# osmocom/osmo-trx

Hardware: AMD Instinct MI355X
Metric: Mbursts/s detect+demod (156.25 sym, 4 SPS) (higher is better)
Workload: dtype f32

## Files before the change

osmo_trx_amd/csrc/trx_capi.cpp:

```cpp
#include <hip/hip_runtime.h>

#include <cmath>
#include <cstdio>
#include <cstdlib>
#include <cstring>
#include <new>
#include <vector>

#include "../../include/trxhip.h"
#include "trx_tables.h"
#include "trx_ctx.h"
#include "trx_launch.h"

extern "C" {

int trxhip_abi_version(void) { return TRXHIP_ABI_VERSION; }

int trxhip_device_count(void)
{
	int n = 0;
	if (hipGetDeviceCount(&n) != hipSuccess)
		return 0;
	return n;
}
// ... 51 lines not shown
	hipDeviceProp_t prop;
	if (hipGetDeviceProperties(&prop, device) != hipSuccess)
		return TRXHIP_ENODEV;

	trxhip_ctx *ctx = new (std::nothrow) trxhip_ctx;
	if (!ctx)
		return TRXHIP_ENOMEM;
	ctx->device = device;
	ctx->n_cu = prop.multiProcessorCount > 0 ? prop.multiProcessorCount : 256;
	ctx->no_unit = trx_unit_masks_match(t) ? 0 : 1;
	ctx->sch_unit = trx_unit_mask_sch_match(t) ? 1 : 0;
	ctx->pool_enabled = getenv("TRXHIP_NO_POOL") ? 0 : 1;
	ctx->nb_enabled = getenv("TRXHIP_NO_NB_KERNEL") ? 0 : 1;
	for (int k = 0; k < 8; k++)
		if (memcmp(&t->dec_taps[k], &t->dec_taps[15 - k], sizeof(float)) != 0)
			ctx->no_sym = 1;
	for (int f = 0; f < 512 && !ctx->no_fast; f++) {
		double sum = 0.0;
		for (int k = 0; k < 8; k++) {
			const int qa = 512 * k + f, qb = 512 * k + (512 - f);
			sum += fabs((double)t->sincv[trx_sincv_swz(qa)]);
			if (qb < TRX_SINCV_LEN)
				sum += fabs((double)t->sincv[trx_sincv_swz(qb)]);
		}
		if (!(sum <= 2.6))
			ctx->no_fast = 1;
	}
	int rc = TRXHIP_OK;
	if (hipMalloc(reinterpret_cast<void **>(&ctx->d_tables), sizeof(trx_tables)) != hipSuccess) {
		ctx->d_tables = nullptr;
		rc = TRXHIP_ENOMEM;
	} else if (hipMemcpy(ctx->d_tables, h_blob, sizeof(trx_tables), hipMemcpyHostToDevice) != hipSuccess) {
		rc = TRXHIP_EIO;
	} else if (!ctx->redo.create()) {
		rc = TRXHIP_ENOMEM;
	} else {
		trx_tx_tables *tx = static_cast<trx_tx_tables *>(malloc(sizeof(trx_tx_tables)));
		if (!tx || trx_tx_tables_generate(tx) != 0)
			rc = TRXHIP_ENOMEM;
		else if (hipMalloc(reinterpret_cast<void **>(&ctx->d_tx_tables), sizeof(trx_tx_tables)) != hipSuccess) {
			ctx->d_tx_tables = nullptr;
			rc = TRXHIP_ENOMEM;
		} else if (hipMemcpy(ctx->d_tx_tables, tx, sizeof(trx_tx_tables), hipMemcpyHostToDevice) != hipSuccess) {
			rc = TRXHIP_EIO;
		}
		free(tx);
	}
	if (rc != TRXHIP_OK) {
		trxhip_destroy(ctx);
		return rc;
	}
	if (hipMalloc(reinterpret_cast<void **>(&ctx->d_pool), TRX_POOL_SLOTS * 64) != hipSuccess ||
	    hipMemset(ctx->d_pool, 0, TRX_POOL_SLOTS * 64) != hipSuccess) {
		if (ctx->d_pool) (void)hipFree(ctx->d_pool);
		ctx->d_pool = nullptr;
	}
	*out = ctx;
	return TRXHIP_OK;
}

int trxhip_create(trxhip_ctx **out, int device)
{
	if (!out)
		return TRXHIP_EINVAL;
	trx_tables *t = static_cast<trx_tables *>(malloc(sizeof(trx_tables)));
	if (!t)
		return TRXHIP_ENOMEM;
	int rc = trx_tables_generate(t) == 0 ? TRXHIP_OK : TRXHIP_EINVAL;
	if (rc == TRXHIP_OK)
		rc = trxhip_create_from_tables(out, device, t, sizeof(trx_tables));
	free(t);
	return rc;
}

void trxhip_destroy(trxhip_ctx *ctx)
{
	if (!ctx)
		return;
	if (hipSetDevice(ctx->device) == hipSuccess) {
		if (ctx->d_tables) (void)hipFree(ctx->d_tables);
		if (ctx->d_pool) (void)hipFree(ctx->d_pool);
		if (ctx->d_tx_tables) (void)hipFree(ctx->d_tx_tables);
		for (float *t : ctx->d_rs_resamp)
			if (t) (void)hipFree(t);
		ctx->redo.destroy();
	}
	delete ctx;
}

int trxhip_set_nb_kernel(trxhip_ctx *ctx, int enabled)
{
	if (!ctx)
		return TRXHIP_EINVAL;
	ctx->nb_enabled = enabled ? 1 : 0;
	return TRXHIP_OK;
}

int trxhip_set_work_pool(trxhip_ctx *ctx, int enabled)
{
	if (!ctx)
		return TRXHIP_EINVAL;
	ctx->pool_enabled = enabled ? 1 : 0;
	return TRXHIP_OK;
}

int trxhip_fast_stats(trxhip_ctx *ctx, uint64_t *out4, int reset)
{
	if (!ctx || !out4)
		return TRXHIP_EINVAL;
	if (with_device(ctx))
		return TRXHIP_EIO;
	unsigned long long v[4] = { 0, 0, 0, 0 };
	if (trx_fast_stats_read(v, reset) != 0)
// ... 89 lines not shown
		return TRXHIP_EIO;
	if (flags & ~(TRXHIP_FLAG_SLICE | TRXHIP_FLAG_EXACT_DEMOD | TRXHIP_FLAG_IDLE_DUMMY | TRXHIP_FLAG_FEW_NB_SLOTS))
		return TRXHIP_EINVAL;
	const bool few_nb = (flags & TRXHIP_FLAG_FEW_NB_SLOTS) != 0;
	flags &= ~TRXHIP_FLAG_FEW_NB_SLOTS;
	if (ctx->no_unit)
		flags |= TRX_IFLAG_NO_UNIT;
	if (ctx->no_sym)
		flags |= TRX_IFLAG_NO_SYM;
	if (ctx->no_fast)
		flags |= TRX_IFLAG_NO_FAST;
	const hipStream_t st = static_cast<hipStream_t>(stream);

	hipStreamCaptureStatus cap = hipStreamCaptureStatusNone;
	const bool capturing = st && hipStreamIsCapturing(st, &cap) == hipSuccess && cap != hipStreamCaptureStatusNone;
	const bool exact = (flags & TRXHIP_FLAG_EXACT_DEMOD) != 0;
	const bool k4 = sps == 4 && burst_len >= 624 && burst_len <= 628;
	const bool common = k4 && burst_len == 625 && d_soft && !d_ebp_in && soft_stride == 148 &&
			    (flags & ~TRXHIP_FLAG_EXACT_DEMOD) == TRXHIP_FLAG_SLICE && !(cf32 && exact);
	const bool split = common && !cf32 && !exact && ctx->nb_enabled && !few_nb && !capturing;
	unsigned *pool = nullptr;
	if (k4 && ctx->d_pool && ctx->pool_enabled && !capturing && n_bursts >= (size_t)ctx->n_cu * 128)
		pool = ctx->d_pool + (size_t)(ctx->pool_next.fetch_add(1u, std::memory_order_relaxed) % TRX_POOL_SLOTS) * 16;

	if (!k4) {
		const int nld = sps == 1 ? 3 : burst_len <= 640 ? 10 : 0;
		return trx_launch_pull(d_iq, cf32, nld, d_params, d_results, d_soft, ctx->d_tables, d_ebp_in, n_bursts, burst_len, sps,
				       threshold, full_scale, soft_stride, flags, ctx->n_cu, st);
	}
	if (split) {
		std::lock_guard<std::mutex> lk(ctx->redo.mu);
		if (trx_redo_lists::slot *sl = ctx->redo.acquire(n_bursts, st)) {
			const int rc = trx_launch_pull4_nb(pool, d_iq, d_params, d_results, d_soft, ctx->d_tables, n_bursts, threshold,
							   full_scale, ctx->n_cu, sl->d, sl->h_left, st);
			ctx->redo.launched(*sl, rc, st);
			return rc;
		}
	}
	return trx_launch_pull4(pool, d_iq, cf32, exact, common, d_params, d_results, d_soft, ctx->d_tables, d_ebp_in, n_bursts,
				burst_len, threshold, full_scale, soft_stride, flags, ctx->n_cu, st);
}

int trxhip_select_diversity_batch(trxhip_ctx *ctx, const int16_t *d_iq_paths, size_t n_bursts, int n_paths, int burst_len, int sps,
				  int16_t *d_iq_sel, float *d_avg_energy, uint8_t *d_path, void *stream)
{
	if (!ctx || n_paths < 1 || n_paths > 8 || (sps != 1 && sps != 4) || burst_len < 1 || burst_len > TRXHIP_MAX_BURST_LEN)
		return TRXHIP_EINVAL;
	{
		const int window = 20 * sps < burst_len ? 20 * sps : burst_len;
		if (4 * (window - 1) >= burst_len)
			return TRXHIP_EINVAL;
	}
	if (n_bursts == 0)
		return TRXHIP_OK;
	if (!d_iq_paths || !d_iq_sel || !d_avg_energy || (reinterpret_cast<uintptr_t>(d_iq_paths) & 3) ||
	    (reinterpret_cast<uintptr_t>(d_iq_sel) & 3))
		return TRXHIP_EINVAL;
	if (with_device(ctx))
		return TRXHIP_EIO;
	return trx_launch_diversity_select(d_iq_paths, n_bursts, n_paths, burst_len, sps, d_iq_sel, d_avg_energy, d_path,
					   static_cast<hipStream_t>(stream));
}

int trxhip_apply_diversity_power(trxhip_ctx *ctx, trxhip_burst_result *d_results, const trxhip_burst_params *d_params,
				 const float *d_avg_energy, size_t n_bursts, float full_scale, void *stream)
{
	if (!ctx || !(full_scale > 0.0f))
// ... 614 lines not shown
```

osmo_trx_amd/csrc/trx_ctx.h:

```cpp
#ifndef TRX_CTX_H
#define TRX_CTX_H
#include <hip/hip_runtime.h>
#include <atomic>
#include <mutex>
#include "../../include/trxhip.h"
#include "trx_tables.h"
#include "trx_tx_tables.h"

#define TRX_POOL_SLOTS 1024
#define TRX_REDO_SLOTS 4

struct trx_redo_lists {
	struct slot {
		unsigned *d = nullptr;
		size_t cap = 0;
		hipEvent_t ev = nullptr;
		bool busy = false;
		unsigned *h_left = nullptr;
		size_t n_last = 0;
	};
	std::mutex mu;
	slot s[TRX_REDO_SLOTS];
	unsigned next = 0;
	unsigned backoff = 0;
// ... 31 lines not shown
			if (hipMalloc(reinterpret_cast<void **>(&sl.d), bytes) != hipSuccess || hipMemsetAsync(sl.d, 0, bytes, stream) != hipSuccess) {
				if (sl.d) (void)hipFree(sl.d);
				sl.d = nullptr;
				return nullptr;
			}
			sl.cap = cap;
		}
		return &sl;
	}
	void launched(slot &sl, int rc, hipStream_t stream)
	{
		if (rc != 0)
			return;
		if (hipEventRecord(sl.ev, stream) == hipSuccess)
			sl.busy = true;
		else
			(void)hipStreamSynchronize(stream);
	}
	void destroy()
	{
		for (slot &sl : s) {
			if (sl.busy) (void)hipEventSynchronize(sl.ev);
			if (sl.ev) (void)hipEventDestroy(sl.ev);
			if (sl.d) (void)hipFree(sl.d);
			if (sl.h_left) (void)hipHostFree(sl.h_left);
		}
	}
};

struct trxhip_ctx {
	int device = 0;
	int n_cu = 0;
	trx_tables *d_tables = nullptr;
	int no_unit = 0;
	int sch_unit = 0;
	int no_sym = 0;
	int no_fast = 0;
	unsigned *d_pool = nullptr;
	int pool_enabled = 1;
	std::atomic<unsigned> pool_next{0u};
	int nb_enabled = 1;
	trx_redo_lists redo;
	trx_tx_tables *d_tx_tables = nullptr;
	std::mutex tx_mu;
	double tx_full_scale = 0.0;
	bool tx_att_valid = false;
	float tx_att_scale[256];
	std::mutex rs_mu;
	float *d_rs_resamp[2] = { nullptr, nullptr };
};

static inline int with_device(const trxhip_ctx *ctx)
{
	return hipSetDevice(ctx->device) == hipSuccess ? 0 : TRXHIP_EIO;
}
#endif
```

osmo_trx_amd/csrc/trx_kernel4.hip:

```cpp
#include <atomic>
#include "trx_device.h"
#include "trx_launch.h"

#include "trx_k4_common.h"

#define K4_CZ_LEN (TRX_CZ_PAD + TRX_CORR_NARROW + TRX_CZ_PAD)
#define K4_SLICE (K4_XS + TRX_DEC_NARROW + K4_CZ_LEN)
#define K4_DROWS (TRX_DELAY_FILTS + 1)
#define K4_PKC_INTS (5 * WAVE)
#define K4_TABLES_FLOATS (TRX_SINCV_LDS + K4_DROWS * TRX_DELAY_HLEN + 2 * 160 + 16 + 2 * LSEQ_TAPS + 8 * LSEQ_NHDR + K4_DROWS * 36 + K4_PKC_INTS)
#define K4_TABLES_BYTES (K4_TABLES_FLOATS * 4)
#define K4_POOL_RING 64
#define K4_POOL_UNSET (-1)
#define K4_POOL_END (-2)
#define K4_NO_BURST 0xffffffffu
#define K4_LDS_TAIL (16 + 4 * K4_POOL_RING)


#ifdef TRX_DIAG
extern "C" int trxhip_diag_read(unsigned long long *out, int reset)
{
	static unsigned long long h[TRX_DIAG_WAVES * 24];
	if (hipMemcpyFromSymbol(h, HIP_SYMBOL(g_trx_diag), sizeof(h)) != hipSuccess) return -1;
	for (int k = 0; k < 32; k++) out[k] = 0;
// ... 895 lines not shown
	DIAG_FLUSH();
}

extern "C" int trx_fast_stats_read(unsigned long long *out4, int reset)
{
	if (hipMemcpyFromSymbol(out4, HIP_SYMBOL(g_trx_fast_stats), 4 * sizeof(unsigned long long)) != hipSuccess)
		return -1;
	if (reset) {
		const unsigned long long z[4] = { 0, 0, 0, 0 };
		if (hipMemcpyToSymbol(HIP_SYMBOL(g_trx_fast_stats), z, sizeof(z)) != hipSuccess)
			return -1;
	}
	return 0;
}

extern "C" int trx_unit_masks_match(const trx_tables *t)
{
	static const unsigned long long want[12] = { TRX_UNIT_NEG_TSC0, TRX_UNIT_NEG_TSC1, TRX_UNIT_NEG_TSC2, TRX_UNIT_NEG_TSC3,
						     TRX_UNIT_NEG_TSC4, TRX_UNIT_NEG_TSC5, TRX_UNIT_NEG_TSC6, TRX_UNIT_NEG_TSC7,
						     TRX_UNIT_NEG_RACH0, TRX_UNIT_NEG_RACH1, TRX_UNIT_NEG_RACH2, TRX_UNIT_NEG_DUMMY };
	for (int s = 0; s < 12; s++)
		if (!((t->unit_ok >> s) & 1u) || t->unit_neg[s] != want[s])
			return 0;
	return 1;
}

#include "trx_kernel_nb.hip"

static inline size_t k4_lds_bytes(bool cf32, bool exact)
{
	return K4_TABLES_BYTES + (size_t)K4_WPB(cf32, exact) * K4_SLICE * sizeof(c32) + K4_LDS_TAIL;
}

extern "C" int trx_launch_pull4_nb(unsigned *d_pool_ctr, const void *d_iq, const trxhip_burst_params *d_params,
				   trxhip_burst_result *d_results, float *d_soft, const trx_tables *d_tab, size_t n_bursts,
				   float thresh, float full_scale, int n_cu, unsigned *d_redo, unsigned *h_left, hipStream_t stream)
{
	if (n_bursts == 0)
		return 0;
	const size_t grid = trx_burst_grid(n_bursts, (size_t)n_cu);
	{
		constexpr auto k = nb_pull4_kernel;
		if (trx_arm_dynamic_lds<k>())
			return TRXHIP_EIO;
		hipLaunchKernelGGL(k, dim3((unsigned)grid), dim3(NB_WPB * WAVE), NB_LDS_BYTES, stream, reinterpret_cast<const uint32_t *>(d_iq),
				   d_params, d_results, d_soft, d_tab, (unsigned)n_bursts, thresh, full_scale, d_pool_ctr, d_redo,
				   thresh * thresh * 0.2f, thresh * thresh * (1.0f / 6.0f), thresh * thresh * (1.0f / 7.0f), thresh * thresh * 0.125f);
	}
	{
		constexpr auto k = burst_pull4_kernel<false, false, true, true>;
		if (trx_arm_dynamic_lds<k>())
			return TRXHIP_EIO;
		hipLaunchKernelGGL(k, dim3((unsigned)n_cu), dim3(K4_WPB(false, false) * WAVE), k4_lds_bytes(false, false), stream, d_iq, d_params,
				   d_results, d_soft, d_tab, (const float4 *)nullptr, (unsigned)n_bursts, 625, thresh, full_scale, 148,
				   TRXHIP_FLAG_SLICE, h_left, d_redo);
	}
	return hipGetLastError() == hipSuccess ? 0 : TRXHIP_EIO;
}

extern "C" int trx_launch_pull4(unsigned *d_pool_ctr, const void *d_iq, int cf32, int exact, int common, const trxhip_burst_params *d_params,
				trxhip_burst_result *d_results, float *d_soft, const trx_tables *d_tab, const float *d_ebp_in, size_t n_bursts,
				int L, float thresh, float full_scale, int soft_stride, int flags, int n_cu, hipStream_t stream)
{
	if (n_bursts == 0)
		return 0;
	const size_t grid = trx_burst_grid(n_bursts, (size_t)n_cu);
	const size_t lds = k4_lds_bytes(cf32, exact);
#define LAUNCH4(CF_, EX_, CM_)                                                                                  \
	do {                                                                                                    \
		constexpr auto k = burst_pull4_kernel<CF_, EX_, CM_>;                                           \
		if (trx_arm_dynamic_lds<k>((int)lds))                                                           \
			return TRXHIP_EIO;                                                                      \
		hipLaunchKernelGGL(k, dim3((unsigned)grid), dim3(K4_WPB(CF_, EX_) * WAVE), lds, stream,         \
				   d_iq, d_params, d_results, d_soft, d_tab, reinterpret_cast<const float4 *>(d_ebp_in), \
				   (unsigned)n_bursts, L, thresh, full_scale, soft_stride, flags, d_pool_ctr, (unsigned *)nullptr); \
	} while (0)
	if (cf32)        { if (exact) LAUNCH4(true, true, false); else if (common) LAUNCH4(true, false, true); else LAUNCH4(true, false, false); }
	else if (common) { if (exact) LAUNCH4(false, true, true); else LAUNCH4(false, false, true); }
	else             { if (exact) LAUNCH4(false, true, false); else LAUNCH4(false, false, false); }
#undef LAUNCH4
// ... 3 lines not shown
```

osmo_trx_amd/csrc/trx_kernel_nb.hip:

```cpp
#include "trx_k4_common.h"
#include "trx_nb_asm.inc"

#define NB_D_LEN    160
#define NB_CZ_LEN   (TRX_CZ_PAD + TRX_CORR_NARROW + TRX_CZ_PAD)
#define NB_SLICE    (K4_XS + NB_D_LEN + NB_CZ_LEN)
#define NB_COMP_ROWS (TRX_DELAY_FILTS + 1)
#define NB_TABLES_FLOATS (TRX_SINCV_LDS + 16 * WAVE + NB_COMP_ROWS * 36 + 16 + 8 * 8 + 5 * WAVE + 5 * WAVE + 2 * 8 * 16)
#define NB_TABLES_BYTES (NB_TABLES_FLOATS * 4)
#define NB_WPB 16
#define NB_POOL_RING 64
#define NB_POOL_UNSET (-1)
#define NB_POOL_END (-2)
#define NB_NO_BURST 0xffffffffu
#define NB_LDS_TAIL (16 + 4 * NB_POOL_RING)
#define NB_LDS_BYTES (NB_TABLES_BYTES + NB_WPB * NB_SLICE * 8 + NB_LDS_TAIL)
#define NB_MAX_TOA 32



typedef float v3f __attribute__((ext_vector_type(3)));
typedef int v4i __attribute__((ext_vector_type(4)));

template <typename T>
__device__ __forceinline__ unsigned lds_addr(const T *p)
{
	return (unsigned)(uintptr_t)(const __attribute__((address_space(3))) T *)p;
}

__global__ void __launch_bounds__(NB_WPB * WAVE)
nb_pull4_kernel(const uint32_t *__restrict__ iq, const trxhip_burst_params *__restrict__ params,
		trxhip_burst_result *__restrict__ results, float *__restrict__ soft, const trx_tables *__restrict__ tab,
		unsigned n_bursts, float thresh, float full_scale, unsigned *__restrict__ pool_ctr, unsigned *__restrict__ redo,
		float gk5, float gk6, float gk7, float gk8)
{
	static_assert(NB_TABLES_BYTES % 16 == 0 && (NB_SLICE * 8) % 16 == 0 && (K4_XS * 8) % 16 == 0 && (NB_D_LEN * 8) % 16 == 0, "16-byte LDS accesses");
	static_assert(NB_LDS_BYTES <= 160 * 1024, "LDS");
	static_assert(NB_ASM_GDEC_OFF == (TRX_SINCV_LDS + 16 * WAVE + NB_COMP_ROWS * 36) * 4, "tools/gen_nb_asm.py: LDS offset of the decimator taps");
	static_assert(NB_ASM_DEC_MAX_NACT == 15 + NB_ASM_CORR_MAX_LEN, "tools/gen_nb_asm.py: DEC and CORR change form at the same window");
	static_assert(NB_ASM_LSEQ_OFF == (NB_TABLES_FLOATS - 2 * 8 * 16) * 4, "tools/gen_nb_asm.py: LDS offset of the training-sequence taps");
	constexpr int NLD = 10;
	extern __shared__ __attribute__((aligned(16))) char smem[];
	const int lane0 = threadIdx.x & (WAVE - 1);
	const int wave = uni((int)(threadIdx.x >> 6));

	float *const sincv = reinterpret_cast<float *>(smem);
	float *const wa4f = sincv + TRX_SINCV_LDS;
	const float4 *const wa4 = reinterpret_cast<const float4 *>(wa4f);
	float *const comp = wa4f + 16 * WAVE;
	float *const gdec = comp + NB_COMP_ROWS * 36;
	float *const lhdr = gdec + 16;
	int *const pkcl = reinterpret_cast<int *>(lhdr + 8 * 8);
	int *const lcn = pkcl + 5 * WAVE;
	c32 *const lseq = reinterpret_cast<c32 *>(lcn + 5 * WAVE);
	c32 *const wbase = reinterpret_cast<c32 *>(smem + NB_TABLES_BYTES) + (size_t)wave * NB_SLICE;
	int *const wg_next = reinterpret_cast<int *>(reinterpret_cast<c32 *>(smem + NB_TABLES_BYTES) + (size_t)NB_WPB * NB_SLICE);
	int *const pool_g = wg_next + 4;
	c32 *const P = wbase;
	c32 *const D = wbase + K4_XS;
	c32 *const cz = D + NB_D_LEN + TRX_CZ_PAD;

	for (int i = threadIdx.x; i < TRX_SINCV_LDS; i += blockDim.x)
		sincv[i] = (i < TRX_SINCV_LEN) ? tab->sincv[i] : 0.0f;
	for (int i = threadIdx.x; i < 16 * WAVE; i += blockDim.x) {
		const int l = i & (WAVE - 1), u = i >> 6;
		const PeakConst pcl = peak_const(l);
		const int q = (u < 8) ? pcl.loA + 512 * (7 - u) : pcl.hiA + 512 * (u - 8);
		wa4f[((u >> 2) * WAVE + l) * 4 + (u & 3)] = (q < TRX_SINCV_LEN) ? tab->sincv[q] : 0.0f;
	}
	for (int i = threadIdx.x; i < NB_COMP_ROWS * 36; i += blockDim.x) {
		const int f = i / 36, j = i % 36;
		comp[i] = (j >= TRX_FUSED_SH) ? tab->comp_filt[f][j - TRX_FUSED_SH] : 0.0f;
	}
	if (threadIdx.x < 16)
		gdec[threadIdx.x] = tab->dec_taps[threadIdx.x];
	if (threadIdx.x < 128)
		lseq[threadIdx.x] = make_float2(tab->seq[TRX_SEQ_TSC0 + (threadIdx.x >> 4)].taps[threadIdx.x & 15].re,
						tab->seq[TRX_SEQ_TSC0 + (threadIdx.x >> 4)].taps[threadIdx.x & 15].im);
	if (threadIdx.x < 64)
		lhdr[threadIdx.x] = reinterpret_cast<const float *>(&tab->seq[TRX_SEQ_TSC0 + (threadIdx.x >> 3)].gain)[threadIdx.x & 7];
	if (threadIdx.x < WAVE) {
		const PeakConst pc0 = peak_const(threadIdx.x);
		pkcl[0 * WAVE + threadIdx.x] = pc0.flA;
		pkcl[1 * WAVE + threadIdx.x] = pc0.loA;
		pkcl[2 * WAVE + threadIdx.x] = pc0.hiA;
		pkcl[3 * WAVE + threadIdx.x] = pc0.offB;
		pkcl[4 * WAVE + threadIdx.x] = pc0.ratio_off;
		lcn[0 * WAVE + threadIdx.x] = pc0.ratio_off * 8;
		lcn[1 * WAVE + threadIdx.x] = (pc0.flA - 8) * 8;
		lcn[2 * WAVE + threadIdx.x] = pc0.offB;
		const int l = threadIdx.x, e = (l - 52) / 3, t = (l - 52) % 3;
		const bool sp = l >= 52;
		lcn[3 * WAVE + l] = 8 * (sp ? (t == 0 ? e : t == 1 ? e + 3 : e - 3) : 4 + 3 * (l < 49 ? l : 49));
		lcn[4 * WAVE + l] = sp ? (e + (t == 2 ? 4 : 0)) * K4_NTP * 4 : -1;
	}
	for (int i = lane0; i < NB_SLICE; i += WAVE)
		wbase[i] = make_float2(0.0f, 0.0f);
	if (threadIdx.x == 0) {
		wg_next[0] = NB_WPB;
		wg_next[1] = 0;
	}
	if (threadIdx.x < NB_POOL_RING)
		pool_g[threadIdx.x] = NB_POOL_UNSET;
	__syncthreads();

	const float fs_db = 6.02059991f * __log2f(full_scale);
	const float thr2 = thresh * thresh;
	const float gc0 = thr2 * 1.0001e-5f;
	int t5pk = 0;
	bool t5_ok = true;
	for (int t = 0; t < 8; t++) {
		const int v = (int)(lhdr[8 * t + 5] * 512.0f);
		t5_ok = t5_ok && v >= -8 && v <= 7 && (float)v == lhdr[8 * t + 5] * 512.0f;
		t5pk |= (v & 15) << (4 * t);
	}
	t5pk = uni(t5pk);
	const unsigned long long e8_addr = reinterpret_cast<unsigned long long>(&tab->edge8[0][0][0]);
	const unsigned n_wg = gridDim.x;
	const unsigned n_groups = (n_bursts + 15u) >> 4;
	const bool pooled = pool_ctr != nullptr;
	const unsigned n_static_groups = pooled ? ((n_groups - (n_groups >> 3)) / n_wg) * n_wg : n_groups;
	const unsigned n_pool_groups = n_groups - n_static_groups;
	const unsigned gq = n_static_groups / n_wg, gr = n_static_groups % n_wg;
	const unsigned my_groups = gq + (blockIdx.x < gr ? 1u : 0u);
	const unsigned base16 = (blockIdx.x * gq + (blockIdx.x < gr ? blockIdx.x : gr)) << 4;
	unsigned items = my_groups << 4;
	if (base16 + items > n_bursts)
		items = (base16 < n_bursts) ? n_bursts - base16 : 0u;
	auto burst_of = [&](unsigned jj) -> unsigned {
		if (jj < items)
			return base16 + jj;
		if (!pooled)
			return NB_NO_BURST;
		const unsigned k = (jj - items) >> 4;
		volatile int *slot = pool_g + (k & (NB_POOL_RING - 1));
		int g;
		while ((g = *slot) == NB_POOL_UNSET)
			__builtin_amdgcn_s_sleep(2);
		g = uni(g);
		if (g < 0)
			return NB_NO_BURST;
		const unsigned bb = ((n_static_groups + (unsigned)g) << 4) + (jj & 15u);
		return bb < n_bursts ? bb : NB_NO_BURST;
	};
	auto pool_draw = [&](unsigned jj, bool ended, int lane) {
		const unsigned k = (jj + 16u - items) >> 4;
		int g = NB_POOL_END;
		if (!ended) {
			unsigned p = 0;
			if (lane == 0)
				p = __hip_atomic_fetch_add(pool_ctr, 1u, __ATOMIC_RELAXED, __HIP_MEMORY_SCOPE_AGENT);
			p = (unsigned)uni((int)p);
			g = (p < n_pool_groups) ? (int)p : NB_POOL_END;
		}
		if (lane == 0) {
			pool_g[(k + NB_POOL_RING / 2) & (NB_POOL_RING - 1)] = NB_POOL_UNSET;
			pool_g[k & (NB_POOL_RING - 1)] = g;
		}
	};

	uint32_t pre_i[NLD];
	uint32_t pre_prm = 0u;
	auto prefetch = [&](unsigned bb, int lane) {
		pre_prm = reinterpret_cast<const uint32_t *>(params)[2 * (size_t)bb];
		const uint32_t *src = iq + (size_t)bb * 625;
		const unsigned ul = (unsigned)lane & 63u;
#pragma unroll
		for (int r = 0; r < NLD - 1; r++)
			pre_i[r] = __builtin_nontemporal_load(src + (unsigned)(r * WAVE) + ul);
		pre_i[NLD - 1] = __builtin_nontemporal_load(src + (unsigned)((NLD - 1) * WAVE) + min(ul, 48u));
	};
	const unsigned b_first = burst_of((unsigned)wave);
	if (b_first != NB_NO_BURST)
		prefetch(b_first, lane0);

	v3f o = { 0.0f, 0.0f, 0.0f };
	int recw = 0;
	bool pend_any = false;
	bool pend_rec = false;
	unsigned pend_b = 0;
	bool left_any = false;
	int q_xr = 0, q_xi = 0, q_es = 0, q_toa = 0, q_s = 0, q_fl = 0, q_b = 0;
	int q_n = 0;
	auto flush_records = [&](const int lane) {
		if (lane < q_n) {
			const float *const h = lhdr + 8 * (q_fl & 0xff);
			const float xr = __int_as_float(q_xr), xi = __int_as_float(q_xi);
			const float a0 = xr * h[2], a1 = xr * h[3], a2 = xi * h[3], a3 = xi * h[2];
			const float amp_re = a0 - a2, amp_im = a1 + a3;
			const float toa = (float)q_toa * 0.001953125f;
			const float energy = __int_as_float(q_es) * 0.0125f;
			const float rssi = fs_db - 3.01029996f * __log2f(energy);
			const float p2 = xi * xi + xr * xr;
			const float C = p2 * h[7];
			const float S = __int_as_float(q_s);
			const float ci = 3.0103f * __log2f(C * __builtin_amdgcn_rcpf(S - C));
			const v4i r0 = { 1, __float_as_int(toa), __float_as_int(amp_re), __float_as_int(amp_im) };
			const v4i r1 = { __float_as_int(ci), __float_as_int(energy), __float_as_int(rssi), q_fl };
			asm volatile("global_store_dwordx4 %0, %1, off\n\t"
				     "global_store_dwordx4 %0, %2, off offset:16\n\t"
				     "s_nop 1"
				     :: "v"(results + (unsigned)q_b), "v"(r0), "v"(r1) : "memory");
		}
		q_n = 0;
	};

	auto demod_general = [&](const int nk, const c32 ampv, const int lane) -> bool {
// ... 87 lines not shown
				dec[hi_i] = cmul(make_float2(sr, si), scale);
		}
		wave_sync();
		auto pick = [&](int i) {
			const float d = reinterpret_cast<const float *>(dec + i)[i & 1];
			return __builtin_amdgcn_fmed3f(fmaf((i & 2) ? -0.5f : 0.5f, d, 0.5f), 0.0f, 1.0f);
		};
		const bool reg = lane >= 2 && lane < 50;
		const int i0 = reg ? 3 * lane - 2 : ((((lane - 54) * 11) >> 5) & 3);
		o.x = pick(i0);
		o.y = pick(reg ? i0 + 1 : 0);
		o.z = pick(reg ? i0 + 2 : 0);
		wave_sync();
		return true;
	};

	DIAG_DECL;
	unsigned j_next = 0, b_next = NB_NO_BURST;
	for (unsigned b = b_first; b != NB_NO_BURST; b = b_next) {
		int lane;
		asm volatile("v_mbcnt_lo_u32_b32 %0, -1, 0\n\tv_mbcnt_hi_u32_b32 %0, -1, %0" : "=v"(lane));
		const int ticket = claim_issue(wg_next);
		const unsigned prm0 = (unsigned)uni((int)pre_prm);
		const unsigned max_toa = prm0 >> 16;
		const int tsc = (prm0 >> 8) & 0xff;
		bool leave = ((prm0 & 0xf8ffu) != (unsigned)TRXHIP_TSC) || (max_toa > NB_MAX_TOA) || !t5_ok;

		c32 *const pload = P + (lane & 3) * PH_A + PH_M0 + (lane >> 2);
		float amax = 0.0f, epart = 0.0f;
#ifdef TRX_DIAG
		DIAG_MARK(12);
		asm volatile("s_waitcnt vmcnt(0)" ::: "memory");
		DIAG_MARK(13);
#endif
		if (!leave) {
#pragma unroll
			for (int r = 0; r < NLD; r++) {
				const int i = r * WAVE + lane;
				if (r < NLD - 1 || i < 625) {
					const c32 v = make_float2((float)(int16_t)(pre_i[r] & 0xffffu), (float)(int16_t)(pre_i[r] >> 16));
					pload[16 * r] = v;
					asm("v_max3_f32 %0, %0, |%1|, |%2|" : "+v"(amax) : "v"(v.x), "v"(v.y));
					if (r < 5)
						epart = fmaf(v.x, v.x, fmaf(v.y, v.y, epart));
				}
			}
		} else {
#pragma unroll
			for (int r = 0; r < NLD; r++)
				asm volatile("" :: "v"(pre_i[r]));
		}
		DIAG_MARK(14);
		if (pend_any) {
			float *const so = soft + (size_t)pend_b * 148;
			int *const rp = reinterpret_cast<int *>(results + pend_b);
			const float oe = o.x;
			asm volatile("s_bfm_b64 exec, 48, 2\n\t"
				     "global_store_dwordx3 %0, %1, %2 offset:16\n\t"
				     "s_mov_b32 exec_lo, 0\n\t"
			     "s_mov_b32 exec_hi, 0x92400000\n\t"
				     "global_store_dword %3, %4, %2\n\t"
				     "s_mov_b64 exec, %8\n\t"
				     "global_store_dword %5, %6, %7\n\t"
				     "s_mov_b64 exec, -1\n\t"
				     "s_nop 0"
				     :: "v"((lane - 2) * 12), "v"(o), "s"(so), "v"((((lane - 54) * 11) >> 5) * 4), "v"(oe), "v"(lane * 4), "v"(recw), "s"(rp),
// ... 159 lines not shown
			continue;
		}
		pend_b = b;
		pend_any = true;
		if (q_n == WAVE)
			flush_records(lane);
		DIAG_MARK(11);
	}
	if (pend_any) {
		int lane;
		asm volatile("v_mbcnt_lo_u32_b32 %0, -1, 0\n\tv_mbcnt_hi_u32_b32 %0, -1, %0" : "=v"(lane));
		float *const so = soft + (size_t)pend_b * 148;
		int *const rp = reinterpret_cast<int *>(results + pend_b);
		const float oe = o.x;
		asm volatile("s_bfm_b64 exec, 48, 2\n\t"
			     "global_store_dwordx3 %0, %1, %2 offset:16\n\t"
		     "s_mov_b32 exec_lo, 0\n\t"
		     "s_mov_b32 exec_hi, 0x92400000\n\t"
			     "global_store_dword %3, %4, %2\n\t"
			     "s_mov_b64 exec, %8\n\t"
			     "global_store_dword %5, %6, %7\n\t"
			     "s_mov_b64 exec, -1\n\t"
			     "s_nop 0"
			     :: "v"((lane - 2) * 12), "v"(o), "s"(so), "v"((((lane - 54) * 11) >> 5) * 4), "v"(oe), "v"(lane * 4), "v"(recw), "s"(rp),
			        "s"(pend_rec ? 0xffull : 0ull)
			     : "memory");
	}
	{
		int lane;
		asm volatile("v_mbcnt_lo_u32_b32 %0, -1, 0\n\tv_mbcnt_hi_u32_b32 %0, -1, %0" : "=v"(lane));
		flush_records(lane);
	}
	DIAG_FLUSH();
	if (pooled) {
		__syncthreads();
		int tid0;
		asm volatile("v_mbcnt_lo_u32_b32 %0, -1, 0\n\tv_mbcnt_hi_u32_b32 %0, -1, %0" : "=v"(tid0));
		if (tid0 == 0 && atomicAdd(wg_next + 1, 1) == 0) {
			const unsigned d = __hip_atomic_fetch_add(pool_ctr + 1, 1u, __ATOMIC_ACQ_REL, __HIP_MEMORY_SCOPE_AGENT);
			if (d == gridDim.x - 1u) {
				__hip_atomic_store(pool_ctr, 0u, __ATOMIC_RELAXED, __HIP_MEMORY_SCOPE_AGENT);
				__hip_atomic_store(pool_ctr + 1, 0u, __ATOMIC_RELEASE, __HIP_MEMORY_SCOPE_AGENT);
			}
		}
	}
}
```

osmo_trx_amd/csrc/trx_launch.h:

```cpp
#ifndef TRX_LAUNCH_H
#define TRX_LAUNCH_H
#include <hip/hip_runtime.h>
#include <stdint.h>
#include "../../include/trxhip.h"
#include "trx_tables.h"
#include "trx_tx_tables.h"

constexpr int trx_arfcn_pchan(int rows, int l)
{
	return rows == 4 ? l : (rows == 1 ? 0 : (rows == 2 ? (l == 0 ? 0 : 3) : (l == 0 ? 1 : (l == 1 ? 0 : 3))));
}

extern "C" {


int trx_launch_pull4(unsigned *d_pool_ctr, const void *d_iq, int cf32, int exact, int common, const trxhip_burst_params *d_params,
		     trxhip_burst_result *d_results, float *d_soft, const trx_tables *d_tab, const float *d_ebp_in, size_t n_bursts,
		     int L, float thresh, float full_scale, int soft_stride, int flags, int n_cu, hipStream_t stream);
int trx_launch_pull4_nb(unsigned *d_pool_ctr, const void *d_iq, const trxhip_burst_params *d_params, trxhip_burst_result *d_results,
			float *d_soft, const trx_tables *d_tab, size_t n_bursts, float thresh, float full_scale, int n_cu,
			unsigned *d_redo, unsigned *h_left, hipStream_t stream);
int trx_launch_pull(const void *d_iq, int cf32, int nld, const trxhip_burst_params *d_params, trxhip_burst_result *d_results,
		    float *d_soft, const trx_tables *d_tab, const float *d_ebp_in, size_t n_bursts, int L, int sps, float thresh,
		    float full_scale, int soft_stride, int flags, int n_cu, hipStream_t stream);
size_t trx_pull_lds_bytes(int L, int waves_per_block);

int trx_fast_stats_read(unsigned long long *out4, int reset);
int trx_unit_masks_match(const trx_tables *t);
int trx_unit_mask_sch_match(const trx_tables *t);

int trx_launch_sch_detect(const float *d_iq, size_t buf_stride, trxhip_burst_result *d_results, const trx_tables *d_tab,
			  size_t n_bufs, int len, int start, int toa_sub, float thresh, int unit_tables, hipStream_t stream);
size_t trx_va_lds_bytes(int L);
int trx_launch_va_demod(const float *d_iq, const trxhip_burst_params *d_params, const trxhip_burst_result *d_detected, float *d_soft,
			int32_t *d_starts, size_t n_bursts, int L, float scale, int soft_stride, int flags, hipStream_t stream);

int trx_launch_pack_trxd(const trxhip_burst_result *d_results, const float *d_soft, int soft_stride, uint8_t *d_pkt,
			 size_t n_bursts, float rssi_offset, hipStream_t stream);
int trx_launch_pack_trxd_wire(const trxhip_burst_result *d_results, const trxhip_burst_params *d_params, const float *d_soft,
			      int soft_stride, const trxhip_trxd_meta *d_meta, uint8_t *d_pkt, int pkt_stride, uint16_t *d_pkt_len,
			      size_t n_bursts, float rssi_offset, hipStream_t stream, trxhip_burst_result *d_results_copy);
int trx_launch_gather_bursts(const unsigned long long *d_src, void *d_dst, size_t n, unsigned dwords, hipStream_t stream);
int trx_launch_convolve(const float *d_x, int x_len, const float *d_h, int h_len, int h_complex, float *d_y, int y_len, int start,
			int len, size_t n_vec, hipStream_t stream);
int trx_launch_convert_short_float(float *d_out, const int16_t *d_in, size_t len, hipStream_t stream);
int trx_launch_convert_float_short(int16_t *d_out, const float *d_in, float scale, size_t len, hipStream_t stream);
int trx_launch_dft_strided(const float *d_in, float *d_out, int m, size_t howmany, size_t istride, size_t ostride, int reverse,
			   hipStream_t stream);
int trx_launch_energy_detect(const float *d_x, size_t n_bursts, int burst_len, unsigned window, float *d_out, hipStream_t stream);
int trx_launch_diversity_select(const int16_t *d_iq_paths, size_t n_bursts, int n_paths, int burst_len, int sps, int16_t *d_iq_sel,
				float *d_avg_energy, uint8_t *d_path, hipStream_t stream);
int trx_launch_diversity_power(trxhip_burst_result *d_res, const trxhip_burst_params *d_params, const float *d_avg_energy,
			       size_t n_bursts, float full_scale, hipStream_t stream);
int trx_launch_delay_vector(const float *d_in, float *d_out, const float *d_delays, const trx_tables *d_tab, size_t n_vec, int len,
// ... 39 lines not shown
```

Baseline: 1079.

## Precompute NB kernel LDS table image once and bulk-copy it per workgroup

Builds the narrowband kernel's LDS table block once at context creation by running a one-off staging kernel and saving the result to a device buffer. Each workgroup of the NB kernel then loads that image with three 16-byte loads per thread and stores it to LDS while the first burst's prefetch is in flight, so the per-element table construction and the t5 packing loop no longer run in every block. This costs an extra device buffer and changes the launch signature. The NB path now fails with EINVAL if the image is missing.

```diff
diff --git a/osmo_trx_amd/csrc/trx_capi.cpp b/osmo_trx_amd/csrc/trx_capi.cpp
--- a/osmo_trx_amd/csrc/trx_capi.cpp
+++ b/osmo_trx_amd/csrc/trx_capi.cpp
@@ -107,6 +107,7 @@
 		rc = TRXHIP_ENOMEM;
 	} else if (hipMemcpy(ctx->d_tables, h_blob, sizeof(trx_tables), hipMemcpyHostToDevice) != hipSuccess) {
 		rc = TRXHIP_EIO;
+	} else if ((rc = trx_nb_lds_image_create(ctx->d_tables, &ctx->d_nb_lds)) != TRXHIP_OK) {
 	} else if (!ctx->redo.create()) {
 		rc = TRXHIP_ENOMEM;
 	} else {
@@ -154,6 +155,7 @@
 		return;
 	if (hipSetDevice(ctx->device) == hipSuccess) {
 		if (ctx->d_tables) (void)hipFree(ctx->d_tables);
+		if (ctx->d_nb_lds) (void)hipFree(ctx->d_nb_lds);
 		if (ctx->d_pool) (void)hipFree(ctx->d_pool);
 		if (ctx->d_tx_tables) (void)hipFree(ctx->d_tx_tables);
 		for (float *t : ctx->d_rs_resamp)
@@ -309,7 +311,7 @@
 		std::lock_guard<std::mutex> lk(ctx->redo.mu);
 		if (trx_redo_lists::slot *sl = ctx->redo.acquire(n_bursts, st)) {
 			const int rc = trx_launch_pull4_nb(pool, d_iq, d_params, d_results, d_soft, ctx->d_tables, n_bursts, threshold,
-							   full_scale, ctx->n_cu, sl->d, sl->h_left, st);
+							   full_scale, ctx->n_cu, sl->d, sl->h_left, ctx->d_nb_lds, st);
 			ctx->redo.launched(*sl, rc, st);
 			return rc;
 		}
diff --git a/osmo_trx_amd/csrc/trx_ctx.h b/osmo_trx_amd/csrc/trx_ctx.h
--- a/osmo_trx_amd/csrc/trx_ctx.h
+++ b/osmo_trx_amd/csrc/trx_ctx.h
@@ -87,6 +87,7 @@
 	int device = 0;
 	int n_cu = 0;
 	trx_tables *d_tables = nullptr;
+	void *d_nb_lds = nullptr;
 	int no_unit = 0;
 	int sch_unit = 0;
 	int no_sym = 0;
diff --git a/osmo_trx_amd/csrc/trx_kernel4.hip b/osmo_trx_amd/csrc/trx_kernel4.hip
--- a/osmo_trx_amd/csrc/trx_kernel4.hip
+++ b/osmo_trx_amd/csrc/trx_kernel4.hip
@@ -951,12 +951,33 @@
 	return K4_TABLES_BYTES + (size_t)K4_WPB(cf32, exact) * K4_SLICE * sizeof(c32) + K4_LDS_TAIL;
 }
 
+extern "C" int trx_nb_lds_image_create(const trx_tables *d_tab, void **d_img)
+{
+	*d_img = nullptr;
+	if (hipMalloc(d_img, NB_TABLES_BYTES) != hipSuccess) {
+		*d_img = nullptr;
+		return TRXHIP_ENOMEM;
+	}
+	constexpr auto k = nb_lds_image_kernel;
+	if (trx_arm_dynamic_lds<k>((int)NB_TABLES_BYTES) == 0) {
+		hipLaunchKernelGGL(k, dim3(1), dim3(NB_WPB * WAVE), NB_TABLES_BYTES, nullptr, d_tab, static_cast<uint4 *>(*d_img));
+		if (hipGetLastError() == hipSuccess && hipStreamSynchronize(nullptr) == hipSuccess)
+			return 0;
+	}
+	(void)hipFree(*d_img);
+	*d_img = nullptr;
+	return TRXHIP_EIO;
+}
+
 extern "C" int trx_launch_pull4_nb(unsigned *d_pool_ctr, const void *d_iq, const trxhip_burst_params *d_params,
 				   trxhip_burst_result *d_results, float *d_soft, const trx_tables *d_tab, size_t n_bursts,
-				   float thresh, float full_scale, int n_cu, unsigned *d_redo, unsigned *h_left, hipStream_t stream)
+				   float thresh, float full_scale, int n_cu, unsigned *d_redo, unsigned *h_left, const void *d_nb_lds,
+				   hipStream_t stream)
 {
 	if (n_bursts == 0)
 		return 0;
+	if (!d_nb_lds)
+		return TRXHIP_EINVAL;
 	const size_t grid = trx_burst_grid(n_bursts, (size_t)n_cu);
 	{
 		constexpr auto k = nb_pull4_kernel;
@@ -964,7 +985,8 @@
 			return TRXHIP_EIO;
 		hipLaunchKernelGGL(k, dim3((unsigned)grid), dim3(NB_WPB * WAVE), NB_LDS_BYTES, stream, reinterpret_cast<const uint32_t *>(d_iq),
 				   d_params, d_results, d_soft, d_tab, (unsigned)n_bursts, thresh, full_scale, d_pool_ctr, d_redo,
-				   thresh * thresh * 0.2f, thresh * thresh * (1.0f / 6.0f), thresh * thresh * (1.0f / 7.0f), thresh * thresh * 0.125f);
+				   thresh * thresh * 0.2f, thresh * thresh * (1.0f / 6.0f), thresh * thresh * (1.0f / 7.0f), thresh * thresh * 0.125f,
+				   static_cast<const uint4 *>(d_nb_lds));
 	}
 	{
 		constexpr auto k = burst_pull4_kernel<false, false, true, true>;
diff --git a/osmo_trx_amd/csrc/trx_kernel_nb.hip b/osmo_trx_amd/csrc/trx_kernel_nb.hip
--- a/osmo_trx_amd/csrc/trx_kernel_nb.hip
+++ b/osmo_trx_amd/csrc/trx_kernel_nb.hip
@@ -5,7 +5,8 @@
 #define NB_CZ_LEN   (TRX_CZ_PAD + TRX_CORR_NARROW + TRX_CZ_PAD)
 #define NB_SLICE    (K4_XS + NB_D_LEN + NB_CZ_LEN)
 #define NB_COMP_ROWS (TRX_DELAY_FILTS + 1)
-#define NB_TABLES_FLOATS (TRX_SINCV_LDS + 16 * WAVE + NB_COMP_ROWS * 36 + 16 + 8 * 8 + 5 * WAVE + 5 * WAVE + 2 * 8 * 16)
+#define NB_T5_ROW 4
+#define NB_TABLES_FLOATS (TRX_SINCV_LDS + 16 * WAVE + NB_COMP_ROWS * 36 + 16 + 8 * 8 + 5 * WAVE + 5 * WAVE + 2 * 8 * 16 + NB_T5_ROW)
 #define NB_TABLES_BYTES (NB_TABLES_FLOATS * 4)
 #define NB_WPB 16
 #define NB_POOL_RING 64
@@ -27,38 +28,17 @@
 	return (unsigned)(uintptr_t)(const __attribute__((address_space(3))) T *)p;
 }
 
-__global__ void __launch_bounds__(NB_WPB * WAVE)
-nb_pull4_kernel(const uint32_t *__restrict__ iq, const trxhip_burst_params *__restrict__ params,
-		trxhip_burst_result *__restrict__ results, float *__restrict__ soft, const trx_tables *__restrict__ tab,
-		unsigned n_bursts, float thresh, float full_scale, unsigned *__restrict__ pool_ctr, unsigned *__restrict__ redo,
-		float gk5, float gk6, float gk7, float gk8)
+__device__ __forceinline__ void nb_stage_tables(char *smem, const trx_tables *__restrict__ tab)
 {
-	static_assert(NB_TABLES_BYTES % 16 == 0 && (NB_SLICE * 8) % 16 == 0 && (K4_XS * 8) % 16 == 0 && (NB_D_LEN * 8) % 16 == 0, "16-byte LDS accesses");
-	static_assert(NB_LDS_BYTES <= 160 * 1024, "LDS");
-	static_assert(NB_ASM_GDEC_OFF == (TRX_SINCV_LDS + 16 * WAVE + NB_COMP_ROWS * 36) * 4, "tools/gen_nb_asm.py: LDS offset of the decimator taps");
-	static_assert(NB_ASM_DEC_MAX_NACT == 15 + NB_ASM_CORR_MAX_LEN, "tools/gen_nb_asm.py: DEC and CORR change form at the same window");
-	static_assert(NB_ASM_LSEQ_OFF == (NB_TABLES_FLOATS - 2 * 8 * 16) * 4, "tools/gen_nb_asm.py: LDS offset of the training-sequence taps");
-	constexpr int NLD = 10;
-	extern __shared__ __attribute__((aligned(16))) char smem[];
-	const int lane0 = threadIdx.x & (WAVE - 1);
-	const int wave = uni((int)(threadIdx.x >> 6));
-
 	float *const sincv = reinterpret_cast<float *>(smem);
 	float *const wa4f = sincv + TRX_SINCV_LDS;
-	const float4 *const wa4 = reinterpret_cast<const float4 *>(wa4f);
 	float *const comp = wa4f + 16 * WAVE;
 	float *const gdec = comp + NB_COMP_ROWS * 36;
 	float *const lhdr = gdec + 16;
 	int *const pkcl = reinterpret_cast<int *>(lhdr + 8 * 8);
 	int *const lcn = pkcl + 5 * WAVE;
 	c32 *const lseq = reinterpret_cast<c32 *>(lcn + 5 * WAVE);
-	c32 *const wbase = reinterpret_cast<c32 *>(smem + NB_TABLES_BYTES) + (size_t)wave * NB_SLICE;
-	int *const wg_next = reinterpret_cast<int *>(reinterpret_cast<c32 *>(smem + NB_TABLES_BYTES) + (size_t)NB_WPB * NB_SLICE);
-	int *const pool_g = wg_next + 4;
-	c32 *const P = wbase;
-	c32 *const D = wbase + K4_XS;
-	c32 *const cz = D + NB_D_LEN + TRX_CZ_PAD;
-
+	int *const t5row = reinterpret_cast<int *>(lseq + 8 * 16);
 	for (int i = threadIdx.x; i < TRX_SINCV_LDS; i += blockDim.x)
 		sincv[i] = (i < TRX_SINCV_LEN) ? tab->sincv[i] : 0.0f;
 	for (int i = threadIdx.x; i < 16 * WAVE; i += blockDim.x) {
@@ -93,28 +73,90 @@
 		lcn[3 * WAVE + l] = 8 * (sp ? (t == 0 ? e : t == 1 ? e + 3 : e - 3) : 4 + 3 * (l < 49 ? l : 49));
 		lcn[4 * WAVE + l] = sp ? (e + (t == 2 ? 4 : 0)) * K4_NTP * 4 : -1;
 	}
-	for (int i = lane0; i < NB_SLICE; i += WAVE)
-		wbase[i] = make_float2(0.0f, 0.0f);
+	__syncthreads();
 	if (threadIdx.x == 0) {
-		wg_next[0] = NB_WPB;
-		wg_next[1] = 0;
-	}
-	if (threadIdx.x < NB_POOL_RING)
-		pool_g[threadIdx.x] = NB_POOL_UNSET;
+		int t5pk = 0;
+		bool t5_ok = true;
+		for (int t = 0; t < 8; t++) {
+			const int v = (int)(lhdr[8 * t + 5] * 512.0f);
+			t5_ok = t5_ok && v >= -8 && v <= 7 && (float)v == lhdr[8 * t + 5] * 512.0f;
+			t5pk |= (v & 15) << (4 * t);
+		}
+		t5row[0] = t5pk;
+		t5row[1] = t5_ok ? 1 : 0;
+		t5row[2] = 0;
+		t5row[3] = 0;
+	}
 	__syncthreads();
-
-	const float fs_db = 6.02059991f * __log2f(full_scale);
-	const float thr2 = thresh * thresh;
-	const float gc0 = thr2 * 1.0001e-5f;
-	int t5pk = 0;
-	bool t5_ok = true;
-	for (int t = 0; t < 8; t++) {
-		const int v = (int)(lhdr[8 * t + 5] * 512.0f);
-		t5_ok = t5_ok && v >= -8 && v <= 7 && (float)v == lhdr[8 * t + 5] * 512.0f;
-		t5pk |= (v & 15) << (4 * t);
-	}
-	t5pk = uni(t5pk);
-	const unsigned long long e8_addr = reinterpret_cast<unsigned long long>(&tab->edge8[0][0][0]);
+}
+
+__global__ void __launch_bounds__(NB_WPB * WAVE)
+nb_lds_image_kernel(const trx_tables *__restrict__ tab, uint4 *__restrict__ d_img)
+{
+	extern __shared__ __attribute__((aligned(16))) char smem[];
+	nb_stage_tables(smem, tab);
+	for (unsigned i = threadIdx.x; i < NB_TABLES_BYTES / 16; i += blockDim.x)
+		d_img[i] = reinterpret_cast<const uint4 *>(smem)[i];
+}
+
+#ifdef TRX_DIAG
+static __device__ unsigned long long g_trx_diag_nb[TRX_DIAG_WAVES * 4];
+extern "C" int trxhip_diag_read_nb_launch(unsigned long long *out, int n_waves)
+{
+	if (n_waves > TRX_DIAG_WAVES) n_waves = TRX_DIAG_WAVES;
+	return hipMemcpyFromSymbol(out, HIP_SYMBOL(g_trx_diag_nb), (size_t)n_waves * 4 * sizeof(unsigned long long)) == hipSuccess ? 0 : -1;
+}
+#endif
+
+__global__ void __launch_bounds__(NB_WPB * WAVE)
+nb_pull4_kernel(const uint32_t *__restrict__ iq, const trxhip_burst_params *__restrict__ params,
+		trxhip_burst_result *__restrict__ results, float *__restrict__ soft, const trx_tables *__restrict__ tab,
+		unsigned n_bursts, float thresh, float full_scale, unsigned *__restrict__ pool_ctr, unsigned *__restrict__ redo,
+		float gk5, float gk6, float gk7, float gk8, const uint4 *__restrict__ nb_img)
+{
+	static_assert(NB_TABLES_BYTES % 16 == 0 && (NB_SLICE * 8) % 16 == 0 && (K4_XS * 8) % 16 == 0 && (NB_D_LEN * 8) % 16 == 0, "16-byte LDS accesses");
+	static_assert(NB_LDS_BYTES <= 160 * 1024, "LDS");
+	static_assert(NB_ASM_GDEC_OFF == (TRX_SINCV_LDS + 16 * WAVE + NB_COMP_ROWS * 36) * 4, "tools/gen_nb_asm.py: LDS offset of the decimator taps");
+	static_assert(NB_ASM_DEC_MAX_NACT == 15 + NB_ASM_CORR_MAX_LEN, "tools/gen_nb_asm.py: DEC and CORR change form at the same window");
+	static_assert(NB_ASM_LSEQ_OFF == (NB_TABLES_FLOATS - NB_T5_ROW - 2 * 8 * 16) * 4, "tools/gen_nb_asm.py: LDS offset of the training-sequence taps");
+	constexpr int NLD = 10;
+#ifdef TRX_DIAG
+	const unsigned long long diag_k0 = __builtin_amdgcn_s_memrealtime();
+	unsigned long long diag_k1 = 0, diag_k2 = 0;
+#endif
+	extern __shared__ __attribute__((aligned(16))) char smem[];
+	const int lane0 = threadIdx.x & (WAVE - 1);
+	const int wave = uni((int)(threadIdx.x >> 6));
+
+	float *const sincv = reinterpret_cast<float *>(smem);
+	float *const wa4f = sincv + TRX_SINCV_LDS;
+	const float4 *const wa4 = reinterpret_cast<const float4 *>(wa4f);
+	float *const comp = wa4f + 16 * WAVE;
+	float *const gdec = comp + NB_COMP_ROWS * 36;
+	float *const lhdr = gdec + 16;
+	int *const pkcl = reinterpret_cast<int *>(lhdr + 8 * 8);
+	int *const lcn = pkcl + 5 * WAVE;
+	c32 *const lseq = reinterpret_cast<c32 *>(lcn + 5 * WAVE);
+	const int *const t5row = reinterpret_cast<const int *>(lseq + 8 * 16);
+	c32 *const wbase = reinterpret_cast<c32 *>(smem + NB_TABLES_BYTES) + (size_t)wave * NB_SLICE;
+	int *const wg_next = reinterpret_cast<int *>(reinterpret_cast<c32 *>(smem + NB_TABLES_BYTES) + (size_t)NB_WPB * NB_SLICE);
+	int *const pool_g = wg_next + 4;
+	c32 *const P = wbase;
+	c32 *const D = wbase + K4_XS;
+	c32 *const cz = D + NB_D_LEN + TRX_CZ_PAD;
+
+	constexpr unsigned NIMG = NB_TABLES_BYTES / 16;
+	static_assert(NIMG > 2 * NB_WPB * WAVE && NIMG <= 3 * NB_WPB * WAVE, "three image loads per thread, the third one partial");
+	const v4i *const img = reinterpret_cast<const v4i *>(nb_img);
+	const v4i im0 = img[threadIdx.x], im1 = img[threadIdx.x + NB_WPB * WAVE];
+	const v4i im2 = img[min(threadIdx.x + 2u * NB_WPB * WAVE, NIMG - 1u)];
+	asm volatile("" ::: "memory");
+	auto store_image = [&]() {
+		reinterpret_cast<v4i *>(smem)[threadIdx.x] = im0;
+		reinterpret_cast<v4i *>(smem)[threadIdx.x + NB_WPB * WAVE] = im1;
+		if (threadIdx.x + 2u * NB_WPB * WAVE < NIMG)
+			reinterpret_cast<v4i *>(smem)[threadIdx.x + 2 * NB_WPB * WAVE] = im2;
+	};
 	const unsigned n_wg = gridDim.x;
 	const unsigned n_groups = (n_bursts + 15u) >> 4;
 	const bool pooled = pool_ctr != nullptr;
@@ -169,9 +211,34 @@
 			pre_i[r] = __builtin_nontemporal_load(src + (unsigned)(r * WAVE) + ul);
 		pre_i[NLD - 1] = __builtin_nontemporal_load(src + (unsigned)((NLD - 1) * WAVE) + min(ul, 48u));
 	};
-	const unsigned b_first = burst_of((unsigned)wave);
-	if (b_first != NB_NO_BURST)
+	const unsigned b_first = ((unsigned)wave < items) ? base16 + (unsigned)wave : NB_NO_BURST;
+	if (b_first != NB_NO_BURST) {
 		prefetch(b_first, lane0);
+		store_image();
+		asm volatile("; image stored under the first burst's prefetch" ::: "memory");
+	} else {
+		store_image();
+		asm volatile("; image stored, no first burst" ::: "memory");
+	}
+	for (int i = lane0; i < NB_SLICE; i += WAVE)
+		wbase[i] = make_float2(0.0f, 0.0f);
+	if (threadIdx.x == 0) {
+		wg_next[0] = NB_WPB;
+		wg_next[1] = 0;
+	}
+	if (threadIdx.x < NB_POOL_RING)
+		pool_g[threadIdx.x] = NB_POOL_UNSET;
+	asm volatile("s_waitcnt lgkmcnt(0)\n\ts_barrier" ::: "memory");
+#ifdef TRX_DIAG
+	diag_k1 = __builtin_amdgcn_s_memrealtime();
+#endif
+
+	const float fs_db = 6.02059991f * __log2f(full_scale);
+	const float thr2 = thresh * thresh;
+	const float gc0 = thr2 * 1.0001e-5f;
+	const int t5pk = uni(t5row[0]);
+	const bool t5_ok = uni(t5row[1]) != 0;
+	const unsigned long long e8_addr = reinterpret_cast<unsigned long long>(&tab->edge8[0][0][0]);
 
 	v3f o = { 0.0f, 0.0f, 0.0f };
 	int recw = 0;
@@ -325,6 +392,8 @@
 		DIAG_MARK(12);
 		asm volatile("s_waitcnt vmcnt(0)" ::: "memory");
 		DIAG_MARK(13);
+		if (!diag_k2)
+			diag_k2 = __builtin_amdgcn_s_memrealtime();
 #endif
 		if (!leave) {
 #pragma unroll
@@ -550,6 +619,14 @@
 		flush_records(lane);
 	}
 	DIAG_FLUSH();
+#ifdef TRX_DIAG
+	if ((threadIdx.x & 63) == 0) {
+		unsigned long long *const g = g_trx_diag_nb + 4 * ((blockIdx.x * 16 + (threadIdx.x >> 6)) % TRX_DIAG_WAVES);
+		g[0] = diag_k0;
+		g[1] = diag_k1;
+		g[2] = diag_k2;
+	}
+#endif
 	if (pooled) {
 		__syncthreads();
 		int tid0;
diff --git a/osmo_trx_amd/csrc/trx_launch.h b/osmo_trx_amd/csrc/trx_launch.h
--- a/osmo_trx_amd/csrc/trx_launch.h
+++ b/osmo_trx_amd/csrc/trx_launch.h
@@ -19,7 +19,8 @@
 		     int L, float thresh, float full_scale, int soft_stride, int flags, int n_cu, hipStream_t stream);
 int trx_launch_pull4_nb(unsigned *d_pool_ctr, const void *d_iq, const trxhip_burst_params *d_params, trxhip_burst_result *d_results,
 			float *d_soft, const trx_tables *d_tab, size_t n_bursts, float thresh, float full_scale, int n_cu,
-			unsigned *d_redo, unsigned *h_left, hipStream_t stream);
+			unsigned *d_redo, unsigned *h_left, const void *d_nb_lds, hipStream_t stream);
+int trx_nb_lds_image_create(const trx_tables *d_tab, void **d_img);
 int trx_launch_pull(const void *d_iq, int cf32, int nld, const trxhip_burst_params *d_params, trxhip_burst_result *d_results,
 		    float *d_soft, const trx_tables *d_tab, const float *d_ebp_in, size_t n_bursts, int L, int sps, float thresh,
 		    float full_scale, int soft_stride, int flags, int n_cu, hipStream_t stream);
```

Result: no change. 1078 (-0.1%).
